# AI4Science-WestlakeU/cindm

Hardware: AMD Instinct MI355X
Metric: design samples/sec (1000-step DDPM, composed U-Nets); rel-err vs CPU ref (higher is better)
Workload: dtype f32; 1 GPU; nbody-2 TemporalUnet1D dim=64 horizon=24 attention, single model, batch 256/GPU, 1000 DDPM steps per design (BASELINE configs[1]); unet_evals_per_design=1000, reverse_steps_per_design=1000, parallelism=dp1 (design-sharded, one all-gather of final designs)

## Files before the change

### cindm_amd/csrc/cindm_hip.hip

```cpp
#include "kernels.h"
#include "kernels_dconv.h"
#include "kernels2d.h"
#include "kernels2d_v2.h"
#include "../../include/cindm_hip.h"

#include <hip/hip_ext.h>
#include <cmath>
#include <cstdio>
#include <cstdlib>
#include <cstring>
#include <map>
#include <mutex>
#include <string>
#include <unordered_map>
#include <vector>

using namespace cindm;

static thread_local std::string g_err;
static int fail(const std::string& m) { g_err = m; return -1; }
#define HIPCHK(x) do { hipError_t e_ = (x); if (e_ != hipSuccess) return fail(std::string(#x) + ": " + hipGetErrorString(e_)); } while (0)
#define REQUIRE(c, msg) do { if (!(c)) return fail(msg); } while (0)

extern "C" int cindm_abi_version(void) { return CINDM_ABI_VERSION; }
// ... 121 lines not shown
    const int mid = h->dims[nres];
    rtb("mid_block1", mid, mid);
    if (d.attention) attn("mid_attn", mid);
    rtb("mid_block2", mid, mid);
    cblock("final_conv.0", dim, dim);
    conv("final_conv.1", dim, d.transition_dim, 1);
    return 0;
}

static const OptDef kUnet1dOpts[] = {
    {"mfma_f32", 0, nullptr, OPT_PACK},
    {"local_gn", 1, "CINDM_LOCAL_GN", OPT_PACK},
    {"attn_site", 1, "CINDM_ATTN_SITE", OPT_PACK},
    {"level0", 1, "CINDM_LEVEL0", OPT_PACK},
    {"level1", 1, "CINDM_LEVEL1", OPT_PACK},
    {"ups_last", 1, "CINDM_UPS_LAST", OPT_PACK},
    {"ups_tail", 1, "CINDM_UPS_TAIL", OPT_PACK},
    {"level_pairs", 1, "CINDM_LEVEL_PAIRS", OPT_PACK},
    {"attn_head", 1, "CINDM_ATTN_HEAD", OPT_PACK},
    {"dconv", 1, "CINDM_DCONV", OPT_PACK},
    {"ws_alias", 1, "CINDM_WS_ALIAS", OPT_PACK},
    {"pingpong", 1, "CINDM_PINGPONG", OPT_PACK},
    {"dresample", 2, "CINDM_DRESAMPLE", OPT_PACK},
    {"dconv2", 1, "CINDM_DCONV2", OPT_PACK},
    {"l2_prefetch", 1, "CINDM_L2_PREFETCH", OPT_PACK},
    {"fuse_gather", 1, nullptr, OPT_PACK},
    {"fuse_update", 1, "CINDM_FUSE_UPDATE", OPT_PACK},
    {"taps", 0, "CINDM_TAPS", OPT_PACK},
    {"recover", 1, nullptr, OPT_RUNTIME},
    {"no_exchange", 0, "CINDM_NO_EXCHANGE", OPT_RUNTIME},
    {"tune", 0, "CINDM_TUNE", OPT_RUNTIME},
    {"stress", 0, "CINDM_STRESS", OPT_PACK},
    {"auto_range", 1, "CINDM_AUTO_RANGE", OPT_PACK},
    {"range_fallback", 0, nullptr, OPT_READONLY},
    {"dbg", 0, "CINDM_DBG", OPT_PACK},
};

static void unet1d_plan(cindm_unet1d* h);
extern "C" int cindm_unet1d_set_option(cindm_unet1d* h, const char* key, int32_t value) {
    const int rc = core_set_option(h, key, value);
    if (rc == 1) {
        h->generation = ++g_generation;
        if (std::string(key) == "tune" && h->finalized) unet1d_plan(h);
    }
    return rc < 0 ? -1 : 0;
}
// ... 597 lines not shown
    if (!identity && !h->packed.count(p + ".residual_conv#h3")) return false;
    const int k0 = x0.C / 128, k1 = x1 ? x1->C / 128 : 0;
    if (w0->second.CinP != (k0 + k1) * 128 || w1->second.CinP != cout || cout % 128) return false;
    return dconv_instantiated(L, k0, k1, !identity) && dconv_instantiated(L, cout / 128, 0, false);
}

static bool dconv2_instantiated(int L, int k0, int k1, bool res, int kb) {
    if (L == 6) return kb == 2 && ((k0 == 1 && k1 == 0 && res) || (k0 == 2 && k1 == 0 && !res) || (k0 == 2 && k1 == 2 && res));
    if (L == 3) return (kb == 4 && ((k0 == 2 && k1 == 0 && res) || (k0 == 4 && k1 == 0 && !res) || (k0 == 4 && k1 == 4 && res))) ||
                       (kb == 2 && k0 == 4 && k1 == 0 && res);
    return false;
}

static Ten emit_rtb_dconv2(Emitter& E, const std::string& p, const Ten& x0, const Ten* x1, int cout) {
    cindm_unet1d* h = E.h;
    const int Bp = (int)E.rows, L = x0.L, S = 48 / L, gw = cout / 8, NT = cout / 32;
    const int tiles = (Bp + S - 1) / S;
    const Packed& w0 = h->packed.at(p + ".blocks.0.block.0");
    const Packed& w1 = h->packed.at(p + ".blocks.1.block.0");
    const bool identity = !h->packed.count(p + ".residual_conv");
    const int k0 = x0.C / 128, k1 = x1 ? x1->C / 128 : 0, kb = cout / 128;
    Ten y0; y0.L = L; y0.C = cout; y0.ld = cout; E.planes(y0);
    Ten out = E.ten(L, cout); E.planes(out);
    unsigned long long* fl = E.xchg((size_t)tiles * NT);
    unsigned long long* xa = gw == 64 ? E.xchg((size_t)tiles * NT * 32) : nullptr;
    unsigned long long* xb = gw == 64 ? E.xchg((size_t)tiles * NT * 32) : nullptr;
    E.need_epoch();
    ++E.launches;
    {
        cindm_unet1d::WReg r{};
        const size_t t0 = w0.sz * 4 / (size_t)NT, t1 = w1.sz * 4 / (size_t)NT;
        int XS = NT / 4;
        while (XS >= 1 && XS < 8 && tiles % (8 / XS) != 0) XS *= 2;
        const bool remap = (XS == 2 || XS == 4) && NT % XS == 0 && tiles % (8 / XS) == 0;
        if (NT % 8 == 0 && !(h->O("tune") & 1)) {
            r.off[0] = w0.off * 4; r.bytes[0] = (unsigned)t0; r.stride[0] = (unsigned)t0;
            if (NT >= 16) { r.off[1] = w0.off * 4 + 8 * t0; r.bytes[1] = (unsigned)t0; r.stride[1] = (unsigned)t0; }
        }
        else if (NT % 8 == 0) { r.off[0] = w0.off * 4; r.bytes[0] = (unsigned)t0; r.stride[0] = (unsigned)t0;
                           r.off[1] = w1.off * 4; r.bytes[1] = (unsigned)t1; r.stride[1] = (unsigned)t1;
                         }
        else { r.off[0] = w0.off * 4; r.bytes[0] = (unsigned)std::min(w0.sz * 4, (size_t)2 << 20); }
        E.pf_issue = p != "downs.3.1";
        Pf pf; E.pf_step(pf, r);
        E.pf_issue = true;
        if (E.dry) { E.drop(y0); return out; }
        Dconv2Args d;
        std::memset(&d, 0, sizeof(d));
        d.pf = pf;
        auto src = [](DSrc& s, const Ten& t) { s.f32 = t.pl ? nullptr : t.p; s.planes = t.pl; s.pstride = t.pst; s.C = t.C; s.ld = t.ld; };
        src(d.src[0], x0); if (x1) src(d.src[1], *x1);
        d.Wa = reinterpret_cast<const uint4*>(E.W(w0)); d.bias_a = E.B(w0); d.ncha = w0.CinP / 128;
        d.Wb = reinterpret_cast<const uint4*>(E.W(w1)); d.bias_b = E.B(w1);
        if (!identity) {
            const Packed& rc = h->packed.at(p + ".residual_conv#h3");
            d.W2 = reinterpret_cast<const uint4*>(E.W(rc)); d.bias2 = E.B(rc);
        } else { d.res = x0.p; d.ldres = x0.ld; }
        d.Bp = Bp; d.N = cout; d.NT = NT; d.gw = gw;
        d.gamma_a = E.V(p + ".blocks.0.block.2.weight"); d.beta_a = E.V(p + ".blocks.0.block.2.bias");
        d.gamma_b = E.V(p + ".blocks.1.block.2.weight"); d.beta_b = E.V(p + ".blocks.1.block.2.bias");
        d.tb = h->ttable + h->tb_off.at(p); d.tb_ld = h->tb_ld; d.t_ptr = E.t_ptr; d.t_imm = E.t_imm;
        d.y0 = y0.pl; d.y0_pstride = y0.pst; d.flags = reinterpret_cast<unsigned*>(fl);
        d.out_f32 = out.p; d.ldo = out.ld; d.out_planes = out.pl; d.out_pstride = out.pst;
        d.xchg_a = xa; d.xchg_b = xb; d.epoch = h->ep(); d.err_flag = h->epoch_dev + 1;
        d.stress = h->O("stress"); d.dbg = h->O("dbg") >= 30 ? h->O("dbg") - 30 : 0;
        d.tune = h->O("tune");
        d.xs = remap ? XS : 0;
        d.ph = E.ph_next("dconv2<" + std::to_string(L) + "," + std::to_string(k0) + "," + std::to_string(k1) + "," + (identity ? "false" : "true") + "," +
                         std::to_string(kb) + "> " + p);
        const dim3 grid((unsigned)NT, (unsigned)tiles);
        const double cin = (double)x0.C + (x1 ? (double)x1->C : 0.0);
        E.prof_begin(4, 2.0 * Bp * L * cout * cin * (5.0 + (identity ? 0.0 : 1.0)) + 2.0 * Bp * L * cout * (double)cout * 5.0);
        if (E.prof) { E.prof->back().gx = grid.x; E.prof->back().gy = grid.y; E.prof->back().nstage = d.ncha + kb; }
#define DC2(L_, K0_, K1_, R_, KB_) KLAUNCH(E, (dconv2_kernel<L_, K0_, K1_, R_, KB_>), grid, dim3(256), 0, d)
        if (L == 6) {
            if (k0 == 1) DC2(6, 1, 0, true, 2);
            else if (k1 == 2) DC2(6, 2, 2, true, 2);
            else DC2(6, 2, 0, false, 2);
        } else {
            if (k0 == 2) DC2(3, 2, 0, true, 4);
            else if (k1 == 4) DC2(3, 4, 4, true, 4);
            else if (kb == 2) DC2(3, 4, 0, true, 2);
            else DC2(3, 4, 0, false, 4);
        }
#undef DC2
        E.prof_end();
        hipError_t e = hipGetLastError();
        if (e != hipSuccess && E.err == hipSuccess) E.err = e;
    }
    E.drop(y0);
    E.tap(p, out);
    return out;
}

static Ten emit_rtb_dconv(Emitter& E, const std::string& p, const Ten& x0, const Ten* x1, int cout) {
    cindm_unet1d* h = E.h;
    const int Bp = (int)E.rows, L = x0.L, S = 48 / L, gw = cout / 8, NT = cout / 32;
    const int tiles = (Bp + S - 1) / S;
    const Packed& w0 = h->packed.at(p + ".blocks.0.block.0");
    const Packed& w1 = h->packed.at(p + ".blocks.1.block.0");
    const bool identity = !h->packed.count(p + ".residual_conv");
    if (h->O("dconv2") && !h->NX() && dconv2_instantiated(L, x0.C / 128, x1 ? x1->C / 128 : 0, !identity, cout / 128) &&
        w0.CinP / 128 == x0.C / 128 + (x1 ? x1->C / 128 : 0))
        return emit_rtb_dconv2(E, p, x0, x1, cout);
// ... 1041 lines not shown
```

### cindm_amd/csrc/kernels_dconv.h

```cpp
#pragma once
#include "kernels.h"
#include <type_traits>

namespace cindm {

__device__ __forceinline__ int spin_bound(const int* err_flag, bool forced_short, int full_log2 = 20) {
    const int seen = err_flag ? uniform_word(err_flag) : 0;
    return (forced_short || seen) ? (1 << 8) : (1 << full_log2);
}

struct DSrc {
    const float* f32;
    const uint4* planes;
    size_t pstride;
    int C, ld;
};

struct DconvArgs {
    DSrc src[2];
    const uint4* W; const float* bias;
    int nch;
    int Bp, N, NT;
    int gw;
    const float* gamma; const float* beta;
// ... 360 lines not shown
            if (sok[q]) a.out2[(size_t)grow[q] * a.ldo2 + gn] = r2[q];
    }
    l2_prefetch_done(a.pf, pfr);
}


struct Dconv2Args {
    DSrc src[2];
    const uint4* Wa; const float* bias_a; int ncha;
    const uint4* Wb; const float* bias_b;
    const uint4* W2; const float* bias2;
    int Bp, N, NT, gw;
    const float* gamma_a; const float* beta_a; const float* gamma_b; const float* beta_b;
    const float* tb; int tb_ld; const int* t_ptr; int t_imm;
    const float* res; int ldres;
    uint4* y0; size_t y0_pstride;
    unsigned* flags;
    float* out_f32; int ldo; uint4* out_planes; size_t out_pstride;
    unsigned long long* xchg_a; unsigned long long* xchg_b; const int* epoch; int* err_flag;
    Pf pf; int stress; int dbg;
    PhaseBuf ph;
    int tune;
    int xs;
};

#ifdef CINDM_KPROF
#define PHK(i) PH(i)
#define PHX(i) do { } while (0)
#else
#define PHK(i) do { } while (0)
#define PHX(i) PH(i)
#endif
template <int L, int KPW0, int KPW1, bool RES, int KPWB>
__global__ __launch_bounds__(256) void dconv2_kernel(const Dconv2Args a) {
    constexpr int T = 5;
    constexpr int S = 48 / L, PB = 16 / S, H = PB - 1, RPAD = (L + 2 * H) * S, NWIN = L + H;
    constexpr int KPWA = KPW0 > KPW1 ? KPW0 : KPW1;
    constexpr int KPWM = KPWA > KPWB ? KPWA : KPWB;
    constexpr int KST = 4 * KPWM;
    constexpr int PLANE_U4 = KST * 4 * RPAD;
    static_assert(L == 3 || L == 6, "3 or 6 positions per sample");
    __shared__ uint4 Img[2][PLANE_U4];
    __shared__ float Red[4][TM * LDR];
    __shared__ uint4 Tile[2 * 48 * 5];

    PH_DECL;
    PH(0);
    const int t_now = step_scalar(a.t_ptr, a.t_imm);
    const unsigned tag = (unsigned)uniform_word(a.epoch);
    const int err_seen = uniform_word(a.err_flag);
    const int tid = threadIdx.x, lane = tid & 63, w = tid >> 6;
    int nt = blockIdx.x, mt = blockIdx.y;
#ifndef CINDM_NO_XCD_REMAP
    if (a.xs > 0) {
        const int XS = a.xs, bl = blockIdx.x + gridDim.x * blockIdx.y, xcd = bl & 7, sl = bl >> 3, q4 = gridDim.x / XS;
        nt = (sl % q4) * XS + (xcd & (XS - 1)); mt = (xcd / XS) + (8 / XS) * (sl / q4);
    }
#endif
    const int b0 = mt * S;
    const int ns = min(S, a.Bp - b0);
    const int n = tid & 31, rq = tid >> 5;
    const int gn = nt * TN + n;
    int grow[6];
    bool sok[6];
#pragma unroll
    for (int q = 0; q < 6; ++q) {
        const int pos = (S == 16) ? (q >> 1) : q;
        const int s = (S == 16) ? rq + 8 * (q & 1) : rq;
        sok[q] = s < ns;
        grow[q] = (b0 + min(s, ns - 1)) * L + pos;
    }

    struct Stg { const uint4* base[3]; size_t kstride, second; int slot[3]; bool f32; };
    auto stg_init = [&](const DSrc& s, Stg& g) {
        g.f32 = s.planes == nullptr;
#pragma unroll
        for (int i = 0; i < 3; ++i) {
            const int item = lane + 64 * i;
            if (!g.f32) {
                const int kq = item / 48, row = item - kq * 48;
                g.base[i] = s.planes + (size_t)mt * (s.C >> 5) * 192 + item;
                g.slot[i] = kq * RPAD + H * S + row;
            } else {
                const int row = item >> 2, kq = item & 3;
                const int sm = row % S, pos = row / S;
                g.base[i] = reinterpret_cast<const uint4*>(s.f32 + (size_t)((b0 + min(sm, ns - 1)) * L + pos) * s.ld + kq * 8);
                g.slot[i] = kq * RPAD + H * S + row;
            }
        }
        g.kstride = g.f32 ? 8 : 192;
        g.second = g.f32 ? 1 : s.pstride;
// ... 12 lines not shown
#pragma unroll
            for (int i = 0; i < 3; ++i) {
                const float4 v0 = __builtin_bit_cast(float4, raw[i][0]), v1 = __builtin_bit_cast(float4, raw[i][1]);
                const float v[8] = {v0.x, v0.y, v0.z, v0.w, v1.x, v1.y, v1.z, v1.w};
                half8 hi, lo;
#pragma unroll
                for (int e = 0; e < 8; ++e) {
                    hi[e] = (_Float16)v[e];
                    lo[e] = (_Float16)((v[e] - (float)hi[e]) * H3_SCALE);
                }
                Img[0][kb + slot[i]] = __builtin_bit_cast(uint4, hi);
                Img[1][kb + slot[i]] = __builtin_bit_cast(uint4, lo);
            }
        }
    };

    Stg g0, g1;
    stg_init(a.src[0], g0);
    uint4 raw0[KPW0][3][2];
#pragma unroll
    for (int j = 0; j < KPW0; ++j) load_raw(g0, j, raw0[j]);

    constexpr int BD = 1;
    half8 wr[BD][T][2][2];
    const uint4* wbase = a.Wa + (size_t)nt * a.ncha * (T * 4) * 256 + tid;
    const uint4* wbase_b = a.Wb + (size_t)nt * KPWB * (T * 4) * 256 + tid;
    auto load_b_tap = [&](const uint4* wb, int ch, int tap, auto slot_c) {
        constexpr int SL = decltype(slot_c)::value;
#if defined(CINDM_ABL) && (CINDM_ABL & 2)
        ch = 0;
#endif
        const uint4* wp = wb + ((size_t)ch * (T * 4) + tap * 4) * 256;
#pragma unroll
        for (int q = 0; q < 4; ++q) wr[SL][tap][q >> 1][q & 1] = __builtin_bit_cast(half8, wp[q * 256]);
    };
    constexpr std::integral_constant<int, 0> SLOT0{};
#pragma unroll
    for (int tap = 0; tap < T; ++tap) load_b_tap(wbase, 0, tap, SLOT0);
    half8 rreg[2][2];
    const uint4* rbase = a.W2 + (size_t)nt * a.ncha * 4 * 256 + tid;
    auto load_r = [&](int ch) {
        if constexpr (RES) {
            const uint4* wp = rbase + (size_t)ch * 4 * 256;
#pragma unroll
            for (int q = 0; q < 4; ++q) rreg[q >> 1][q & 1] = __builtin_bit_cast(half8, wp[q * 256]);
        }
    };
    load_r(0);
    uint4 raw1[KPW1 > 0 ? KPW1 : 1][3][2];
    if constexpr (KPW1 > 0) {
        stg_init(a.src[1], g1);
#pragma unroll
        for (int j = 0; j < KPW1; ++j) load_raw(g1, j, raw1[j]);
    }
    __builtin_amdgcn_sched_barrier(0);
    const int spin_cap = (a.dbg == 9 || err_seen) ? (1 << 8) : (1 << 20);
    const float gam_a = a.gamma_a[gn], bet_a = a.beta_a[gn], gam_b = a.gamma_b[gn], bet_b = a.beta_b[gn];
    const float bias_a_ld = (a.bias_a ? a.bias_a : a.gamma_a)[gn], bias_b_ld = (a.bias_b ? a.bias_b : a.gamma_a)[gn];
    const float tbv_ld = a.tb ? a.tb[(size_t)t_now * a.tb_ld + gn] : bias_a_ld;
    const float bias_a = a.bias_a ? bias_a_ld : 0.f, bias_b = a.bias_b ? bias_b_ld : 0.f, tbv = a.tb ? tbv_ld : 0.f;
    float bias2 = 0.f;
    if constexpr (RES) { const float b2 = (a.bias2 ? a.bias2 : a.gamma_a)[gn]; bias2 = a.bias2 ? b2 : 0.f; }
    float rs[6] = {0.f, 0.f, 0.f, 0.f, 0.f, 0.f};
    if constexpr (!RES) {
#pragma unroll
        for (int q = 0; q < 6; ++q) rs[q] = a.res[(size_t)grow[q] * a.ldres + gn];
    }
    __builtin_amdgcn_sched_barrier(0);
    PH(1);

    if constexpr (H > 0) {
        const uint4 z = {0u, 0u, 0u, 0u};
        for (int i = lane; i < KPWM * 4 * 2 * H * S; i += 64) {
            const int blk = i / (2 * H * S), r = i - blk * (2 * H * S);
            const int ks = 4 * (blk >> 2) + w, kq = blk & 3;
            const int row = r < H * S ? r : (L + H) * S + (r - H * S);
            Img[0][(ks * 4 + kq) * RPAD + row] = z;
            Img[1][(ks * 4 + kq) * RPAD + row] = z;
        }
    }

    f32x4 accM[3][2], accL[3][2], accRM[3][2], accRL[3][2];
    auto zero_acc = [&]() {
#pragma unroll
        for (int i = 0; i < 3; ++i)
#pragma unroll
            for (int j = 0; j < 2; ++j) { accM[i][j] = (f32x4){0.f, 0.f, 0.f, 0.f}; accL[i][j] = (f32x4){0.f, 0.f, 0.f, 0.f}; }
    };
    zero_acc();
#pragma unroll
    for (int i = 0; i < 3; ++i)
#pragma unroll
        for (int j = 0; j < 2; ++j) { accRM[i][j] = (f32x4){0.f, 0.f, 0.f, 0.f}; accRL[i][j] = (f32x4){0.f, 0.f, 0.f, 0.f}; }

    auto kstep = [&](const uint4* wb, int j, int chn, auto pf, auto ride, auto slot_c) {
        constexpr bool PF = decltype(pf)::value;
        constexpr bool RIDE = decltype(ride)::value;
        constexpr int SL = decltype(slot_c)::value;
        const int base = ((4 * j + w) * 4 + (lane >> 4)) * RPAD + (lane & 15);
        half8 fh[NWIN], fl[NWIN];
#pragma unroll
        for (int p = 0; p < NWIN; ++p) {
            fh[p] = __builtin_bit_cast(half8, Img[0][base + p * S]);
            fl[p] = __builtin_bit_cast(half8, Img[1][base + p * S]);
        }
#pragma unroll
        for (int tap = 0; tap < T; ++tap) {
#pragma unroll
            for (int mb = 0; mb < 3; ++mb) {
                const int p = mb * PB + tap - 2 + H;
                if (p < 0 || p >= NWIN) continue;
#if defined(CINDM_ABL) && (CINDM_ABL & 1)
#pragma unroll
                for (int nb = 0; nb < 2; ++nb)
#pragma unroll
                    for (int pl = 0; pl < 2; ++pl) {
                        const uint4 u = __builtin_bit_cast(uint4, wr[SL][tap][nb][pl]);
                        asm volatile("" :: "v"(u.x), "v"(u.y), "v"(u.z), "v"(u.w));
                    }
                {
                    const uint4 u = __builtin_bit_cast(uint4, fh[p]), u2 = __builtin_bit_cast(uint4, fl[p]);
                    asm volatile("" :: "v"(u.x), "v"(u.y), "v"(u.z), "v"(u.w), "v"(u2.x), "v"(u2.y), "v"(u2.z), "v"(u2.w));
                }
#else
#pragma unroll
                for (int nb = 0; nb < 2; ++nb) {
                    accM[mb][nb] = __builtin_amdgcn_mfma_f32_16x16x32_f16(fh[p], wr[SL][tap][nb][0], accM[mb][nb], 0, 0, 0);
                    accL[mb][nb] = __builtin_amdgcn_mfma_f32_16x16x32_f16(fh[p], wr[SL][tap][nb][1], accL[mb][nb], 0, 0, 0);
                }
#pragma unroll
                for (int nb = 0; nb < 2; ++nb)
                    accL[mb][nb] = __builtin_amdgcn_mfma_f32_16x16x32_f16(fl[p], wr[SL][tap][nb][0], accL[mb][nb], 0, 0, 0);
#endif
            }
            if constexpr (RIDE) if (tap == 2) {
#pragma unroll
                for (int mb = 0; mb < 3; ++mb) {
                    const int p = mb * PB + H;
#pragma unroll
                    for (int nb = 0; nb < 2; ++nb) {
                        accRM[mb][nb] = __builtin_amdgcn_mfma_f32_16x16x32_f16(fh[p], rreg[nb][0], accRM[mb][nb], 0, 0, 0);
                        accRL[mb][nb] = __builtin_amdgcn_mfma_f32_16x16x32_f16(fh[p], rreg[nb][1], accRL[mb][nb], 0, 0, 0);
                    }
#pragma unroll
                    for (int nb = 0; nb < 2; ++nb)
                        accRL[mb][nb] = __builtin_amdgcn_mfma_f32_16x16x32_f16(fl[p], rreg[nb][0], accRL[mb][nb], 0, 0, 0);
                }
                if constexpr (PF) load_r(chn);
            }
            if constexpr (PF) {
                load_b_tap(wb, chn, tap, slot_c);
                __builtin_amdgcn_sched_barrier(0);
            }
        }
    };
    constexpr std::true_type YES{};
    constexpr std::false_type NO{};
    constexpr std::integral_constant<bool, RES> RIDE_A{};
    if constexpr (KPW1 == 0) {
#pragma unroll
        for (int j = 0; j < KPW0 - 1; ++j) { store_raw(g0.f32, g0.slot, j, raw0[j]); PHK(2 + 2 * j); kstep(wbase, j, j + 1, YES, RIDE_A, SLOT0); PHK(3 + 2 * j); }
        store_raw(g0.f32, g0.slot, KPW0 - 1, raw0[KPW0 - 1]);
        PHK(2 + 2 * (KPW0 - 1));
        kstep(wbase, KPW0 - 1, 0, NO, RIDE_A, SLOT0);
        PHK(3 + 2 * (KPW0 - 1));
    } else {
#pragma unroll
        for (int j = 0; j < KPW0; ++j) { store_raw(g0.f32, g0.slot, j, raw0[j]); kstep(wbase, j, j + 1, YES, RIDE_A, SLOT0); }
#pragma unroll
        for (int j = 0; j < KPW1 - 1; ++j) { store_raw(g1.f32, g1.slot, j, raw1[j]); kstep(wbase, j, KPW0 + j + 1, YES, RIDE_A, SLOT0); }
        store_raw(g1.f32, g1.slot, KPW1 - 1, raw1[KPW1 - 1]);
        kstep(wbase, KPW1 - 1, 0, NO, RIDE_A, SLOT0);
    }
    PHX(2);
    PfRegs pfr;
#pragma unroll
    for (int k = 0; k < PF_REGIONS; ++k) pfr.v[k][0] = pfr.v[k][1] = 0u;
    auto issue_b = [&]() {
#pragma unroll
        for (int tap = 0; tap < T; ++tap) load_b_tap(wbase_b, 0, tap, SLOT0);
        __builtin_amdgcn_sched_barrier(0);
    };

    auto reduce_to = [&](const f32x4 (&m)[3][2], const f32x4 (&l)[3][2], float bs, float (&v)[6]) {
#pragma unroll
        for (int mb = 0; mb < 3; ++mb)
#pragma unroll
            for (int nb = 0; nb < 2; ++nb)
#pragma unroll
                for (int rg = 0; rg < 4; ++rg)
                    Red[w][(mb * 16 + (lane >> 4) * 4 + rg) * LDR + nb * 16 + (lane & 15)] = m[mb][nb][rg] + l[mb][nb][rg] * H3_INV;
        __syncthreads();
#pragma unroll
        for (int q = 0; q < 6; ++q) {
            const int r = rq + 8 * q;
            v[q] = ((Red[0][r * LDR + n] + Red[1][r * LDR + n]) + (Red[2][r * LDR + n] + Red[3][r * LDR + n])) + bs;
        }
    };
    constexpr int NSAMP = (S == 16) ? 2 : 1;
    const int gwt = a.gw < TN ? a.gw : TN;
    const float cnt = (float)(L * gwt);
    auto gn_mish = [&](const float (&v)[6], unsigned long long* xchg, float gam, float bet, float (&y)[6], auto phb, auto after_xchg) {
        constexpr int PHB = decltype(phb)::value;
        (void)PHB;
        float mean[NSAMP], rstd[NSAMP];
#pragma unroll
        for (int js = 0; js < NSAMP; ++js) {
            float s1 = 0.f;
#pragma unroll
            for (int pos = 0; pos < L; ++pos) s1 += v[(S == 16) ? 2 * pos + js : pos];
            s1 = row16_sum(s1);
            if (gwt == 32) s1 = xsum16(s1);
            const float m = s1 / cnt;
            float s2 = 0.f;
#pragma unroll
            for (int pos = 0; pos < L; ++pos) { const float d = v[(S == 16) ? 2 * pos + js : pos] - m; s2 += d * d; }
            s2 = row16_sum(s2);
            if (gwt == 32) s2 = xsum16(s2);
            mean[js] = m; rstd[js] = s2;
        }
        if (a.gw == 64) {
            stress_delay(a.stress, 1u);
            const int sbase = ((mt * a.NT + nt) * 16) * 2, pbase = ((mt * a.NT + (nt ^ 1)) * 16) * 2;
#pragma unroll
            for (int js = 0; js < NSAMP; ++js) {
                const int s = (S == 16) ? rq + 8 * js : rq;
                if (n == 0) {
                    const unsigned long long q0 = ((unsigned long long)tag << 32) | __builtin_bit_cast(unsigned, mean[js]);
                    const unsigned long long q1 = ((unsigned long long)tag << 32) | __builtin_bit_cast(unsigned, rstd[js]);
                    __hip_atomic_store(xchg + sbase + s * 2, q0, __ATOMIC_RELAXED, __HIP_MEMORY_SCOPE_AGENT);
                    __hip_atomic_store(xchg + sbase + s * 2 + 1, q1, __ATOMIC_RELAXED, __HIP_MEMORY_SCOPE_AGENT);
                }
            }
            stress_delay(a.stress, 2u);
            PHX(PHB);
            unsigned long long gq[NSAMP][2];
            {
                int spins = 0;
                while (true) {
                    bool ok = true;
#pragma unroll
                    for (int js = 0; js < NSAMP; ++js) {
                        const int s = (S == 16) ? rq + 8 * js : rq;
                        gq[js][0] = __hip_atomic_load(xchg + pbase + s * 2, __ATOMIC_RELAXED, __HIP_MEMORY_SCOPE_AGENT);
// ... 2 lines not shown
#pragma unroll
                    for (int js = 0; js < NSAMP; ++js) ok = ok & ((unsigned)(gq[js][0] >> 32) == tag) & ((unsigned)(gq[js][1] >> 32) == tag);
                    if (__all(ok)) break;
                    if (++spins > spin_cap) { if (lane == 0) atomicExch(a.err_flag, 1); break; }
                    __builtin_amdgcn_s_sleep(2);
                }
            }
#pragma unroll
            for (int js = 0; js < NSAMP; ++js) {
                const unsigned long long q0 = gq[js][0], q1 = gq[js][1];
                const float mp = __builtin_bit_cast(float, (unsigned)q0), M2p = __builtin_bit_cast(float, (unsigned)q1);
                const float m = 0.5f * (mean[js] + mp);
                const float d0 = mean[js] - m, d1 = mp - m;
                mean[js] = m;
                rstd[js] = (rstd[js] + M2p) + cnt * (d0 * d0 + d1 * d1);
            }
            PHX(PHB + 1);
        }
        after_xchg();
        const float cnt_all = a.gw == 64 ? 2.f * cnt : cnt;
#pragma unroll
        for (int js = 0; js < NSAMP; ++js) rstd[js] = 1.0f / sqrtf(rstd[js] / cnt_all + 1e-5f);
#pragma unroll
        for (int q = 0; q < 6; ++q) {
            const int js = (S == 16) ? (q & 1) : 0;
            y[q] = mish_f((v[q] - mean[js]) * rstd[js] * gam + bet);
        }
    };
    constexpr int TP = 20;
    auto planes_to_tile = [&](const float (&y)[6]) {
        uint32_t* tw = reinterpret_cast<uint32_t*>(Tile);
#pragma unroll
        for (int q = 0; q < 6; ++q) {
            const int r = rq + 8 * q;
            const _Float16 hi = (_Float16)y[q];
            const _Float16 lo = (_Float16)((y[q] - (float)hi) * H3_SCALE);
            const uint32_t own = (uint32_t)__builtin_bit_cast(uint16_t, hi) | ((uint32_t)__builtin_bit_cast(uint16_t, lo) << 16);
            const uint32_t nbr = (uint32_t)__builtin_amdgcn_update_dpp(0, (int)own, 0xB1, 0xf, 0xf, false);
            const bool odd = n & 1;
            const uint32_t word = odd ? ((nbr >> 16) | (own & 0xffff0000u)) : ((own & 0xffffu) | (nbr << 16));
            tw[(odd ? 48 * TP : 0) + r * TP + (n >> 1)] = word;
        }
    };

    float v[6], y[6];
    stress_delay(a.stress, 3u);
    reduce_to(accM, accL, bias_a, v);
    PHX(3);
    gn_mish(v, a.xchg_a, gam_a, bet_a, y, std::integral_constant<int, 4>{}, [&]() {});
#pragma unroll
    for (int q = 0; q < 6; ++q) y[q] += tbv;
    planes_to_tile(y);
    stress_delay(a.stress, 4u);
    __syncthreads();
    {
        const uint32_t* tw = reinterpret_cast<const uint32_t*>(Tile);
        const size_t plane_bytes = a.y0_pstride * 16;
        const auto rsrc = __builtin_amdgcn_make_buffer_rsrc(reinterpret_cast<void*>(a.y0), 0, (unsigned)(2 * plane_bytes), 0x00020000);
        auto store_item = [&](int i) {
            const int pl = i >= 192 ? 1 : 0, within = i - pl * 192;
            const int kq = within / 48, row = within - kq * 48;
            const uint4 t4 = *reinterpret_cast<const uint4*>(tw + pl * 48 * TP + row * TP + kq * 4);
            const unsigned off = (unsigned)(pl * plane_bytes + (((size_t)mt * a.NT + nt) * 192 + within) * 16);
            typedef unsigned int u32x4 __attribute__((ext_vector_type(4)));
            __builtin_amdgcn_raw_buffer_store_b128(__builtin_bit_cast(u32x4, t4), rsrc, off, 0, 16);
        };
        for (int i = tid; i < 384; i += 256) store_item(i);
        PHX(6);
        asm volatile("s_waitcnt vmcnt(0)" ::: "memory");
        stress_delay(a.stress, 6u);
        __syncthreads();
        if (tid == 0 && !(a.dbg == 9 && (nt & 1)))
            __hip_atomic_store(a.flags + 2 * ((size_t)mt * a.NT + nt), tag, __ATOMIC_RELAXED, __HIP_MEMORY_SCOPE_AGENT);
        PHX(7);
        issue_b();
        if (a.tune & 1) l2_prefetch(a.pf, pfr);
    }
    float r2[6] = {0.f, 0.f, 0.f, 0.f, 0.f, 0.f};
    if constexpr (RES) { reduce_to(accRM, accRL, bias2, r2); __syncthreads(); }
    PHX(8);

    constexpr int YB = KPWB < 2 ? KPWB : 2;
    uint4 rawb[YB][3][2];
    int slotb[3];
#pragma unroll
    for (int i = 0; i < 3; ++i) { const int item = lane + 64 * i, kq = item / 48, row = item - kq * 48; slotb[i] = kq * RPAD + H * S + row; }
    const size_t y0_plane_bytes = a.y0_pstride * 16;
    const auto y0_rsrc = __builtin_amdgcn_make_buffer_rsrc(reinterpret_cast<void*>(a.y0), 0, (unsigned)(2 * y0_plane_bytes), 0x00020000);
    auto fetch_y0 = [&](int j, uint4 (&dst)[3][2]) {
#pragma unroll
        for (int i = 0; i < 3; ++i) {
            const unsigned off = (unsigned)((((size_t)mt * a.NT + 4 * j + w) * 192 + lane + 64 * i) * 16);
            dst[i][0] = __builtin_bit_cast(uint4, __builtin_amdgcn_raw_buffer_load_b128(y0_rsrc, off, 0, 16));
            dst[i][1] = __builtin_bit_cast(uint4, __builtin_amdgcn_raw_buffer_load_b128(y0_rsrc, off + (unsigned)y0_plane_bytes, 0, 16));
        }
    };
    {
        stress_delay(a.stress, 7u);
        int spins = 0;
        const int spin_max = spin_cap;
        while (true) {
            unsigned fw[KPWB];
#pragma unroll
            for (int j = 0; j < KPWB; ++j)
                fw[j] = __hip_atomic_load(a.flags + 2 * ((size_t)mt * a.NT + 4 * j + w), __ATOMIC_RELAXED, __HIP_MEMORY_SCOPE_AGENT);
            bool ok = true;
#pragma unroll
            for (int j = 0; j < KPWB; ++j) ok = ok & (fw[j] == tag);
            if (ok) break;
            if (++spins > spin_max) { if (lane == 0) atomicExch(a.err_flag, 1); break; }
            __builtin_amdgcn_s_sleep(1);
        }
        asm volatile("" ::: "memory");
        PHX(9);
#pragma unroll
        for (int j = 0; j < YB; ++j) fetch_y0(j, rawb[j]);
        __builtin_amdgcn_sched_barrier(0);
    }
    zero_acc();
    auto kb_step = [&](auto jc) {
        constexpr int j = decltype(jc)::value;
        constexpr std::integral_constant<int, j % BD> slot{};
        store_raw(false, slotb, j, rawb[j % YB]);
        if (j + YB < KPWB) fetch_y0(j + YB, rawb[j % YB]);
        __builtin_amdgcn_sched_barrier(0);
        if constexpr (j + BD < KPWB) kstep(wbase_b, j, j + BD, YES, NO, slot);
        else kstep(wbase_b, j, 0, NO, NO, slot);
        __builtin_amdgcn_sched_barrier(0);
    };
    kb_step(std::integral_constant<int, 0>{});
    if constexpr (KPWB > 1) kb_step(std::integral_constant<int, 1>{});
    if constexpr (KPWB > 2) kb_step(std::integral_constant<int, 2>{});
    if constexpr (KPWB > 3) kb_step(std::integral_constant<int, 3>{});
    static_assert(KPWB <= 4, "phase B: at most four k-steps per wave");
    PHX(10);
    if (!(a.tune & 1)) l2_prefetch(a.pf, pfr);

    stress_delay(a.stress, 8u);
    reduce_to(accM, accL, bias_b, v);
    PHX(11);
    gn_mish(v, a.xchg_b, gam_b, bet_b, y, std::integral_constant<int, 12>{}, [&]() {});
#pragma unroll
    for (int q = 0; q < 6; ++q) y[q] += RES ? r2[q] : rs[q];
    if (a.out_f32 && a.pf.wt) {
        float ta[4] = {y[0], y[1], y[2], y[3]}, tb[4] = {y[4], y[5], 0.f, 0.f};
        quad_transpose4(ta, lane);
        quad_transpose4(tb, lane);
        const int j = lane & 3;
        const size_t c4 = (size_t)(gn & ~3);
        auto row_ok = [&](int q, int& g) { const int pos = (S == 16) ? (q >> 1) : q; const int sm = (S == 16) ? rq + 8 * (q & 1) : rq; g = (b0 + min(sm, ns - 1)) * L + pos; return sm < ns; };
        int g0; const bool ok0 = row_ok(j, g0);
        if (ok0) st_out4(a.out_f32, (size_t)g0 * a.ldo + c4, make_float4(ta[0], ta[1], ta[2], ta[3]), 1);
        if (j < 2) { int g1; if (row_ok(4 + j, g1)) st_out4(a.out_f32, (size_t)g1 * a.ldo + c4, make_float4(tb[0], tb[1], tb[2], tb[3]), 1); }
    } else {
#pragma unroll
        for (int q = 0; q < 6; ++q)
            if (a.out_f32 && sok[q]) st_out(a.out_f32, (size_t)grow[q] * a.ldo + gn, y[q], 0);
    }
    if (a.out_planes) {
        __syncthreads();
        planes_to_tile(y);
        __syncthreads();
        const uint32_t* tw = reinterpret_cast<const uint32_t*>(Tile);
        for (int i = tid; i < 384; i += 256) {
            const int pl = i >= 192 ? 1 : 0, within = i - pl * 192;
            const int kq = within / 48, row = within - kq * 48;
            const uint4 t4 = *reinterpret_cast<const uint4*>(tw + pl * 48 * TP + row * TP + kq * 4);
            st_out4(a.out_planes, pl * a.out_pstride + ((size_t)mt * a.NT + nt) * 192 + within, t4, a.pf.wt);
        }
    }
    PHX(14);
    l2_prefetch_done(a.pf, pfr);
    PH_FLUSH(a.ph);
}


struct DresArgs {
    const float* x; int ld;
    const uint4* W; const float* bias; int nch;
    int Bp, N, NT;
    float* out_f32; int ldo;
    uint4* out_planes; size_t out_pstride;
    Pf pf;
    PhaseBuf ph;
    int xs;
};

template <bool UP, int KPW, int NH>
__global__ __launch_bounds__(256) void dresample_kernel(const DresArgs a) {
// ... 455 lines not shown
```

Before: 845.0 samples/s.

## Split L=3 dconv2 blocks into 16-column halves with cross-block GroupNorm exchange

Adds an NH=2 form of the fused double-conv kernel for the L=3, single-source, 1x1-residual case. Each 32-column tile is split across two workgroups, doubling the grid when it stays within 256 blocks. The halves combine GroupNorm statistics through a tagged atomic exchange in global memory, and the final output is written by a keeper half using partner values sent via new exchange buffers. The aim is more parallelism for an under-filled layer, at the cost of extra global-memory spin-waits and exchange traffic.

```diff
diff --git a/cindm_amd/csrc/cindm_hip.hip b/cindm_amd/csrc/cindm_hip.hip
--- a/cindm_amd/csrc/cindm_hip.hip
+++ b/cindm_amd/csrc/cindm_hip.hip
@@ -167,6 +167,7 @@
     {"ws_alias", 1, "CINDM_WS_ALIAS", OPT_PACK},
     {"pingpong", 1, "CINDM_PINGPONG", OPT_PACK},
     {"dresample", 2, "CINDM_DRESAMPLE", OPT_PACK},
+    {"dconv2_split", 1, "CINDM_DCONV2_SPLIT", OPT_PACK},
     {"dconv2", 1, "CINDM_DCONV2", OPT_PACK},
     {"l2_prefetch", 1, "CINDM_L2_PREFETCH", OPT_PACK},
     {"fuse_gather", 1, nullptr, OPT_PACK},
@@ -810,17 +811,21 @@
     const int k0 = x0.C / 128, k1 = x1 ? x1->C / 128 : 0, kb = cout / 128;
     Ten y0; y0.L = L; y0.C = cout; y0.ld = cout; E.planes(y0);
     Ten out = E.ten(L, cout); E.planes(out);
-    unsigned long long* fl = E.xchg((size_t)tiles * NT);
-    unsigned long long* xa = gw == 64 ? E.xchg((size_t)tiles * NT * 32) : nullptr;
-    unsigned long long* xb = gw == 64 ? E.xchg((size_t)tiles * NT * 32) : nullptr;
+    const bool split = h->O("dconv2_split") && L == 3 && k0 == 4 && k1 == 0 && kb == 2 && !identity && gw == 32 && 2 * NT * tiles <= 256;
+    const int NH = split ? 2 : 1;
+    unsigned long long* fl = E.xchg((size_t)tiles * NT * NH);
+    unsigned long long* xa = gw == 64 || split ? E.xchg((size_t)tiles * NT * NH * 32) : nullptr;
+    unsigned long long* xb = gw == 64 || split ? E.xchg((size_t)tiles * NT * NH * 32) : nullptr;
+    unsigned long long* xv = split ? E.xchg((size_t)tiles * NT * NH * 3 * 128) : nullptr;
+    unsigned long long* xr = split ? E.xchg((size_t)tiles * NT * NH * 3 * 128) : nullptr;
     E.need_epoch();
     ++E.launches;
     {
         cindm_unet1d::WReg r{};
         const size_t t0 = w0.sz * 4 / (size_t)NT, t1 = w1.sz * 4 / (size_t)NT;
-        int XS = NT / 4;
+        int XS = NH * NT / 4;
         while (XS >= 1 && XS < 8 && tiles % (8 / XS) != 0) XS *= 2;
-        const bool remap = (XS == 2 || XS == 4) && NT % XS == 0 && tiles % (8 / XS) == 0;
+        const bool remap = (XS == 2 || XS == 4) && (NH * NT) % XS == 0 && tiles % (8 / XS) == 0 && (!split || XS == 4);
         if (NT % 8 == 0 && !(h->O("tune") & 1)) {
             r.off[0] = w0.off * 4; r.bytes[0] = (unsigned)t0; r.stride[0] = (unsigned)t0;
             if (NT >= 16) { r.off[1] = w0.off * 4 + 8 * t0; r.bytes[1] = (unsigned)t0; r.stride[1] = (unsigned)t0; }
@@ -854,9 +859,10 @@
         d.stress = h->O("stress"); d.dbg = h->O("dbg") >= 30 ? h->O("dbg") - 30 : 0;
         d.tune = h->O("tune");
         d.xs = remap ? XS : 0;
+        d.xchg_v = xv; d.xchg_r = xr;
         d.ph = E.ph_next("dconv2<" + std::to_string(L) + "," + std::to_string(k0) + "," + std::to_string(k1) + "," + (identity ? "false" : "true") + "," +
                          std::to_string(kb) + "> " + p);
-        const dim3 grid((unsigned)NT, (unsigned)tiles);
+        const dim3 grid((unsigned)(NH * NT), (unsigned)tiles);
         const double cin = (double)x0.C + (x1 ? (double)x1->C : 0.0);
         E.prof_begin(4, 2.0 * Bp * L * cout * cin * (5.0 + (identity ? 0.0 : 1.0)) + 2.0 * Bp * L * cout * (double)cout * 5.0);
         if (E.prof) { E.prof->back().gx = grid.x; E.prof->back().gy = grid.y; E.prof->back().nstage = d.ncha + kb; }
@@ -868,6 +874,7 @@
         } else {
             if (k0 == 2) DC2(3, 2, 0, true, 4);
             else if (k1 == 4) DC2(3, 4, 4, true, 4);
+            else if (kb == 2 && split) KLAUNCH(E, (dconv2_kernel<3, 4, 0, true, 2, 2>), grid, dim3(256), 0, d);
             else if (kb == 2) DC2(3, 4, 0, true, 2);
             else DC2(3, 4, 0, false, 4);
         }
diff --git a/cindm_amd/csrc/kernels_dconv.h b/cindm_amd/csrc/kernels_dconv.h
--- a/cindm_amd/csrc/kernels_dconv.h
+++ b/cindm_amd/csrc/kernels_dconv.h
@@ -406,7 +406,21 @@
     PhaseBuf ph;
     int tune;
     int xs;
+    unsigned long long* xchg_v; unsigned long long* xchg_r;
 };
+
+__device__ __forceinline__ void merge_halves(float m0, float M0, float m1, float M1, float cnt, float& mean, float& M2) {
+    const float m = 0.5f * (m0 + m1);
+    const float d0 = m0 - m, d1 = m1 - m;
+    mean = m;
+    M2 = (M0 + M1) + cnt * (d0 * d0 + d1 * d1);
+}
+__device__ __forceinline__ void row_pair(float own, bool odd_row, float& v0, float& v1) {
+    float p, q;
+    permlane16_pair(own, p, q);
+    const float other = __builtin_bit_cast(unsigned, p) == __builtin_bit_cast(unsigned, own) ? q : p;
+    v0 = odd_row ? other : own; v1 = odd_row ? own : other;
+}
 
 #ifdef CINDM_KPROF
 #define PHK(i) PH(i)
@@ -415,7 +429,7 @@
 #define PHK(i) do { } while (0)
 #define PHX(i) PH(i)
 #endif
-template <int L, int KPW0, int KPW1, bool RES, int KPWB>
+template <int L, int KPW0, int KPW1, bool RES, int KPWB, int NH = 1>
 __global__ __launch_bounds__(256) void dconv2_kernel(const Dconv2Args a) {
     constexpr int T = 5;
     constexpr int S = 48 / L, PB = 16 / S, H = PB - 1, RPAD = (L + 2 * H) * S, NWIN = L + H;
@@ -424,6 +438,8 @@
     constexpr int KST = 4 * KPWM;
     constexpr int PLANE_U4 = KST * 4 * RPAD;
     static_assert(L == 3 || L == 6, "3 or 6 positions per sample");
+    constexpr int NBW = 2 / NH, TNW = TN / NH, RQN = 256 / TNW, NQ = TM / RQN;
+    static_assert(NH == 1 || (NH == 2 && L == 3 && RES && KPW1 == 0), "16-column form: L = 3 blocks with a riding 1x1, one source");
     __shared__ uint4 Img[2][PLANE_U4];
     __shared__ float Red[4][TM * LDR];
     __shared__ uint4 Tile[2 * 48 * 5];
@@ -441,16 +457,22 @@
         nt = (sl % q4) * XS + (xcd & (XS - 1)); mt = (xcd / XS) + (8 / XS) * (sl / q4);
     }
 #endif
+    int hb = 0;
+    if constexpr (NH == 2) {
+        const int hx = nt;
+        hb = hx & 1;
+        nt = a.xs == 4 ? ((hx >> 1) & 1) * 2 + ((hx >> 2) & 1) + 4 * (hx >> 3) : hx >> 1;
+    }
     const int b0 = mt * S;
     const int ns = min(S, a.Bp - b0);
-    const int n = tid & 31, rq = tid >> 5;
-    const int gn = nt * TN + n;
-    int grow[6];
-    bool sok[6];
-#pragma unroll
-    for (int q = 0; q < 6; ++q) {
-        const int pos = (S == 16) ? (q >> 1) : q;
-        const int s = (S == 16) ? rq + 8 * (q & 1) : rq;
+    const int n = tid & (TNW - 1), rq = tid / TNW;
+    const int gn = nt * TN + hb * TNW + n;
+    int grow[NQ];
+    bool sok[NQ];
+#pragma unroll
+    for (int q = 0; q < NQ; ++q) {
+        const int pos = (S == 16 && NH == 1) ? (q >> 1) : q;
+        const int s = (S == 16 && NH == 1) ? rq + 8 * (q & 1) : rq;
         sok[q] = s < ns;
         grow[q] = (b0 + min(s, ns - 1)) * L + pos;
     }
@@ -509,7 +531,7 @@
     for (int j = 0; j < KPW0; ++j) load_raw(g0, j, raw0[j]);
 
     constexpr int BD = 1;
-    half8 wr[BD][T][2][2];
+    half8 wr[BD][T][NBW][2];
     const uint4* wbase = a.Wa + (size_t)nt * a.ncha * (T * 4) * 256 + tid;
     const uint4* wbase_b = a.Wb + (size_t)nt * KPWB * (T * 4) * 256 + tid;
     auto load_b_tap = [&](const uint4* wb, int ch, int tap, auto slot_c) {
@@ -519,18 +541,18 @@
 #endif
         const uint4* wp = wb + ((size_t)ch * (T * 4) + tap * 4) * 256;
 #pragma unroll
-        for (int q = 0; q < 4; ++q) wr[SL][tap][q >> 1][q & 1] = __builtin_bit_cast(half8, wp[q * 256]);
+        for (int q = 0; q < 2 * NBW; ++q) wr[SL][tap][q >> 1][q & 1] = __builtin_bit_cast(half8, wp[(NH == 2 ? hb * 2 + q : q) * 256]);
     };
     constexpr std::integral_constant<int, 0> SLOT0{};
 #pragma unroll
     for (int tap = 0; tap < T; ++tap) load_b_tap(wbase, 0, tap, SLOT0);
-    half8 rreg[2][2];
+    half8 rreg[NBW][2];
     const uint4* rbase = a.W2 + (size_t)nt * a.ncha * 4 * 256 + tid;
     auto load_r = [&](int ch) {
         if constexpr (RES) {
             const uint4* wp = rbase + (size_t)ch * 4 * 256;
 #pragma unroll
-            for (int q = 0; q < 4; ++q) rreg[q >> 1][q & 1] = __builtin_bit_cast(half8, wp[q * 256]);
+            for (int q = 0; q < 2 * NBW; ++q) rreg[q >> 1][q & 1] = __builtin_bit_cast(half8, wp[(NH == 2 ? hb * 2 + q : q) * 256]);
         }
     };
     load_r(0);
@@ -548,10 +570,14 @@
     const float bias_a = a.bias_a ? bias_a_ld : 0.f, bias_b = a.bias_b ? bias_b_ld : 0.f, tbv = a.tb ? tbv_ld : 0.f;
     float bias2 = 0.f;
     if constexpr (RES) { const float b2 = (a.bias2 ? a.bias2 : a.gamma_a)[gn]; bias2 = a.bias2 ? b2 : 0.f; }
-    float rs[6] = {0.f, 0.f, 0.f, 0.f, 0.f, 0.f};
+    float rs[NQ];
+#pragma unroll
+    for (int q = 0; q < NQ; ++q) rs[q] = 0.f;
+    float gam_bp = 0.f, bet_bp = 0.f;
+    if constexpr (NH == 2) { const int gnp = nt * TN + (hb ^ 1) * TNW + n; gam_bp = a.gamma_b[gnp]; bet_bp = a.beta_b[gnp]; }
     if constexpr (!RES) {
 #pragma unroll
-        for (int q = 0; q < 6; ++q) rs[q] = a.res[(size_t)grow[q] * a.ldres + gn];
+        for (int q = 0; q < NQ; ++q) rs[q] = a.res[(size_t)grow[q] * a.ldres + gn];
     }
     __builtin_amdgcn_sched_barrier(0);
     PH(1);
@@ -567,18 +593,18 @@
         }
     }
 
-    f32x4 accM[3][2], accL[3][2], accRM[3][2], accRL[3][2];
+    f32x4 accM[3][NBW], accL[3][NBW], accRM[3][NBW], accRL[3][NBW];
     auto zero_acc = [&]() {
 #pragma unroll
         for (int i = 0; i < 3; ++i)
 #pragma unroll
-            for (int j = 0; j < 2; ++j) { accM[i][j] = (f32x4){0.f, 0.f, 0.f, 0.f}; accL[i][j] = (f32x4){0.f, 0.f, 0.f, 0.f}; }
+            for (int j = 0; j < NBW; ++j) { accM[i][j] = (f32x4){0.f, 0.f, 0.f, 0.f}; accL[i][j] = (f32x4){0.f, 0.f, 0.f, 0.f}; }
     };
     zero_acc();
 #pragma unroll
     for (int i = 0; i < 3; ++i)
 #pragma unroll
-        for (int j = 0; j < 2; ++j) { accRM[i][j] = (f32x4){0.f, 0.f, 0.f, 0.f}; accRL[i][j] = (f32x4){0.f, 0.f, 0.f, 0.f}; }
+        for (int j = 0; j < NBW; ++j) { accRM[i][j] = (f32x4){0.f, 0.f, 0.f, 0.f}; accRL[i][j] = (f32x4){0.f, 0.f, 0.f, 0.f}; }
 
     auto kstep = [&](const uint4* wb, int j, int chn, auto pf, auto ride, auto slot_c) {
         constexpr bool PF = decltype(pf)::value;
@@ -599,7 +625,7 @@
                 if (p < 0 || p >= NWIN) continue;
 #if defined(CINDM_ABL) && (CINDM_ABL & 1)
 #pragma unroll
-                for (int nb = 0; nb < 2; ++nb)
+                for (int nb = 0; nb < NBW; ++nb)
 #pragma unroll
                     for (int pl = 0; pl < 2; ++pl) {
                         const uint4 u = __builtin_bit_cast(uint4, wr[SL][tap][nb][pl]);
@@ -611,12 +637,12 @@
                 }
 #else
 #pragma unroll
-                for (int nb = 0; nb < 2; ++nb) {
+                for (int nb = 0; nb < NBW; ++nb) {
                     accM[mb][nb] = __builtin_amdgcn_mfma_f32_16x16x32_f16(fh[p], wr[SL][tap][nb][0], accM[mb][nb], 0, 0, 0);
                     accL[mb][nb] = __builtin_amdgcn_mfma_f32_16x16x32_f16(fh[p], wr[SL][tap][nb][1], accL[mb][nb], 0, 0, 0);
                 }
 #pragma unroll
-                for (int nb = 0; nb < 2; ++nb)
+                for (int nb = 0; nb < NBW; ++nb)
                     accL[mb][nb] = __builtin_amdgcn_mfma_f32_16x16x32_f16(fl[p], wr[SL][tap][nb][0], accL[mb][nb], 0, 0, 0);
 #endif
             }
@@ -625,12 +651,12 @@
                 for (int mb = 0; mb < 3; ++mb) {
                     const int p = mb * PB + H;
 #pragma unroll
-                    for (int nb = 0; nb < 2; ++nb) {
+                    for (int nb = 0; nb < NBW; ++nb) {
                         accRM[mb][nb] = __builtin_amdgcn_mfma_f32_16x16x32_f16(fh[p], rreg[nb][0], accRM[mb][nb], 0, 0, 0);
                         accRL[mb][nb] = __builtin_amdgcn_mfma_f32_16x16x32_f16(fh[p], rreg[nb][1], accRL[mb][nb], 0, 0, 0);
                     }
 #pragma unroll
-                    for (int nb = 0; nb < 2; ++nb)
+                    for (int nb = 0; nb < NBW; ++nb)
                         accRL[mb][nb] = __builtin_amdgcn_mfma_f32_16x16x32_f16(fl[p], rreg[nb][0], accRL[mb][nb], 0, 0, 0);
                 }
                 if constexpr (PF) load_r(chn);
@@ -669,44 +695,115 @@
         __builtin_amdgcn_sched_barrier(0);
     };
 
-    auto reduce_to = [&](const f32x4 (&m)[3][2], const f32x4 (&l)[3][2], float bs, float (&v)[6]) {
+    auto reduce_to = [&](const f32x4 (&m)[3][NBW], const f32x4 (&l)[3][NBW], float bs, float (&v)[NQ]) {
 #pragma unroll
         for (int mb = 0; mb < 3; ++mb)
 #pragma unroll
-            for (int nb = 0; nb < 2; ++nb)
+            for (int nb = 0; nb < NBW; ++nb)
 #pragma unroll
                 for (int rg = 0; rg < 4; ++rg)
                     Red[w][(mb * 16 + (lane >> 4) * 4 + rg) * LDR + nb * 16 + (lane & 15)] = m[mb][nb][rg] + l[mb][nb][rg] * H3_INV;
         __syncthreads();
 #pragma unroll
-        for (int q = 0; q < 6; ++q) {
-            const int r = rq + 8 * q;
+        for (int q = 0; q < NQ; ++q) {
+            const int r = rq + RQN * q;
             v[q] = ((Red[0][r * LDR + n] + Red[1][r * LDR + n]) + (Red[2][r * LDR + n] + Red[3][r * LDR + n])) + bs;
         }
     };
-    constexpr int NSAMP = (S == 16) ? 2 : 1;
+    constexpr int NSAMP = (S == 16 && NH == 1) ? 2 : 1;
     const int gwt = a.gw < TN ? a.gw : TN;
     const float cnt = (float)(L * gwt);
-    auto gn_mish = [&](const float (&v)[6], unsigned long long* xchg, float gam, float bet, float (&y)[6], auto phb, auto after_xchg) {
+    const bool halfwise = NH == 2 || a.gw == 32;
+    const float cnt_h = (float)(L * 16);
+    const bool keeper = NH == 2 && (rq >> 3) == hb;
+    const int xslot = (mt * a.NT + nt) * 2;
+    const int lidx = (rq & 7) * 16 + n;
+    float ypart[NQ];
+    float r2[NQ];
+#pragma unroll
+    for (int q = 0; q < NQ; ++q) { ypart[q] = 0.f; r2[q] = 0.f; }
+    auto gn_mish = [&](const float (&v)[NQ], unsigned long long* xchg, float gam, float bet, float (&y)[NQ], auto phb, auto after_xchg, auto lines) {
         constexpr int PHB = decltype(phb)::value;
+        constexpr bool LINES = decltype(lines)::value;
         (void)PHB;
         float mean[NSAMP], rstd[NSAMP];
 #pragma unroll
         for (int js = 0; js < NSAMP; ++js) {
             float s1 = 0.f;
 #pragma unroll
-            for (int pos = 0; pos < L; ++pos) s1 += v[(S == 16) ? 2 * pos + js : pos];
+            for (int pos = 0; pos < L; ++pos) s1 += v[(S == 16 && NH == 1) ? 2 * pos + js : pos];
             s1 = row16_sum(s1);
-            if (gwt == 32) s1 = xsum16(s1);
-            const float m = s1 / cnt;
+            if (!halfwise && gwt == 32) s1 = xsum16(s1);
+            const float m = s1 / (halfwise ? cnt_h : cnt);
             float s2 = 0.f;
 #pragma unroll
-            for (int pos = 0; pos < L; ++pos) { const float d = v[(S == 16) ? 2 * pos + js : pos] - m; s2 += d * d; }
+            for (int pos = 0; pos < L; ++pos) { const float d = v[(S == 16 && NH == 1) ? 2 * pos + js : pos] - m; s2 += d * d; }
             s2 = row16_sum(s2);
-            if (gwt == 32) s2 = xsum16(s2);
+            if (!halfwise && gwt == 32) s2 = xsum16(s2);
             mean[js] = m; rstd[js] = s2;
-        }
-        if (a.gw == 64) {
+            if (NH == 1 && halfwise) {
+                const bool odd_row = (n >> 4) & 1;
+                float m0, m1, M0, M1;
+                row_pair(m, odd_row, m0, m1);
+                row_pair(s2, odd_row, M0, M1);
+                merge_halves(m0, M0, m1, M1, cnt_h, mean[js], rstd[js]);
+            }
+        }
+        if constexpr (NH == 2) {
+            stress_delay(a.stress, 1u);
+            const int sbase = (xslot + hb) * 32, pbase = (xslot + (hb ^ 1)) * 32;
+            if (n == 0) {
+                const unsigned long long q0 = ((unsigned long long)tag << 32) | __builtin_bit_cast(unsigned, mean[0]);
+                const unsigned long long q1 = ((unsigned long long)tag << 32) | __builtin_bit_cast(unsigned, rstd[0]);
+                __hip_atomic_store(xchg + sbase + rq * 2, q0, __ATOMIC_RELAXED, __HIP_MEMORY_SCOPE_AGENT);
+                __hip_atomic_store(xchg + sbase + rq * 2 + 1, q1, __ATOMIC_RELAXED, __HIP_MEMORY_SCOPE_AGENT);
+            }
+            if constexpr (LINES) if (!keeper) {
+#pragma unroll
+                for (int q = 0; q < NQ; ++q)
+                    __hip_atomic_store(a.xchg_v + ((size_t)(xslot + hb) * NQ + q) * 128 + lidx, ((unsigned long long)tag << 32) | __builtin_bit_cast(unsigned, v[q]),
+                                       __ATOMIC_RELAXED, __HIP_MEMORY_SCOPE_AGENT);
+            }
+            stress_delay(a.stress, 2u);
+            PHX(PHB);
+            const bool wantl = LINES && keeper;
+            unsigned long long gq[2], gv[NQ], gr[NQ];
+#pragma unroll
+            for (int q = 0; q < NQ; ++q) gv[q] = gr[q] = 0ull;
+            {
+                int spins = 0;
+                while (true) {
+                    gq[0] = __hip_atomic_load(xchg + pbase + rq * 2, __ATOMIC_RELAXED, __HIP_MEMORY_SCOPE_AGENT);
+                    gq[1] = __hip_atomic_load(xchg + pbase + rq * 2 + 1, __ATOMIC_RELAXED, __HIP_MEMORY_SCOPE_AGENT);
+                    bool ok = ((unsigned)(gq[0] >> 32) == tag) & ((unsigned)(gq[1] >> 32) == tag);
+                    if (wantl) {
+#pragma unroll
+                        for (int q = 0; q < NQ; ++q) {
+                            const size_t o = ((size_t)(xslot + (hb ^ 1)) * NQ + q) * 128 + lidx;
+                            gv[q] = __hip_atomic_load(a.xchg_v + o, __ATOMIC_RELAXED, __HIP_MEMORY_SCOPE_AGENT);
+                            gr[q] = __hip_atomic_load(a.xchg_r + o, __ATOMIC_RELAXED, __HIP_MEMORY_SCOPE_AGENT);
+                        }
+#pragma unroll
+                        for (int q = 0; q < NQ; ++q) ok = ok & ((unsigned)(gv[q] >> 32) == tag) & ((unsigned)(gr[q] >> 32) == tag);
+                    }
+                    if (__all(ok)) break;
+                    if (++spins > spin_cap) { if (lane == 0) atomicExch(a.err_flag, 1); break; }
+                    __builtin_amdgcn_s_sleep(2);
+                }
+            }
+            const float mp = __builtin_bit_cast(float, (unsigned)gq[0]), M2p = __builtin_bit_cast(float, (unsigned)gq[1]);
+            const float mo = mean[0], M2o = rstd[0];
+            if (hb == 0) merge_halves(mo, M2o, mp, M2p, cnt_h, mean[0], rstd[0]);
+            else merge_halves(mp, M2p, mo, M2o, cnt_h, mean[0], rstd[0]);
+            if (wantl) {
+                const float rs_ = 1.0f / sqrtf(rstd[0] / cnt + 1e-5f);
+#pragma unroll
+                for (int q = 0; q < NQ; ++q)
+                    ypart[q] = mish_f((__builtin_bit_cast(float, (unsigned)gv[q]) - mean[0]) * rs_ * gam_bp + bet_bp) + __builtin_bit_cast(float, (unsigned)gr[q]);
+            }
+            PHX(PHB + 1);
+        }
+        if (NH == 1 && a.gw == 64) {
             stress_delay(a.stress, 1u);
             const int sbase = ((mt * a.NT + nt) * 16) * 2, pbase = ((mt * a.NT + (nt ^ 1)) * 16) * 2;
 #pragma unroll
@@ -755,17 +852,17 @@
 #pragma unroll
         for (int js = 0; js < NSAMP; ++js) rstd[js] = 1.0f / sqrtf(rstd[js] / cnt_all + 1e-5f);
 #pragma unroll
-        for (int q = 0; q < 6; ++q) {
-            const int js = (S == 16) ? (q & 1) : 0;
+        for (int q = 0; q < NQ; ++q) {
+            const int js = (S == 16 && NH == 1) ? (q & 1) : 0;
             y[q] = mish_f((v[q] - mean[js]) * rstd[js] * gam + bet);
         }
     };
     constexpr int TP = 20;
-    auto planes_to_tile = [&](const float (&y)[6]) {
+    auto planes_to_tile = [&](const float (&y)[NQ]) {
         uint32_t* tw = reinterpret_cast<uint32_t*>(Tile);
 #pragma unroll
-        for (int q = 0; q < 6; ++q) {
-            const int r = rq + 8 * q;
+        for (int q = 0; q < NQ; ++q) {
+            const int r = rq + RQN * q;
             const _Float16 hi = (_Float16)y[q];
             const _Float16 lo = (_Float16)((y[q] - (float)hi) * H3_SCALE);
             const uint32_t own = (uint32_t)__builtin_bit_cast(uint16_t, hi) | ((uint32_t)__builtin_bit_cast(uint16_t, lo) << 16);
@@ -776,13 +873,21 @@
         }
     };
 
-    float v[6], y[6];
+    auto tile_item = [&](int i, int& pl, int& within, int& kq, int& row) {
+        constexpr int PER = 192 / NH;
+        pl = i >= PER ? 1 : 0;
+        const int wl = i - pl * PER;
+        kq = wl / 48; row = wl - kq * 48;
+        within = (NH == 2 ? 2 * hb * 48 : 0) + wl;
+    };
+
+    float v[NQ], y[NQ];
     stress_delay(a.stress, 3u);
     reduce_to(accM, accL, bias_a, v);
     PHX(3);
-    gn_mish(v, a.xchg_a, gam_a, bet_a, y, std::integral_constant<int, 4>{}, [&]() {});
-#pragma unroll
-    for (int q = 0; q < 6; ++q) y[q] += tbv;
+    gn_mish(v, a.xchg_a, gam_a, bet_a, y, std::integral_constant<int, 4>{}, [&]() {}, NO);
+#pragma unroll
+    for (int q = 0; q < NQ; ++q) y[q] += tbv;
     planes_to_tile(y);
     stress_delay(a.stress, 4u);
     __syncthreads();
@@ -791,26 +896,31 @@
         const size_t plane_bytes = a.y0_pstride * 16;
         const auto rsrc = __builtin_amdgcn_make_buffer_rsrc(reinterpret_cast<void*>(a.y0), 0, (unsigned)(2 * plane_bytes), 0x00020000);
         auto store_item = [&](int i) {
-            const int pl = i >= 192 ? 1 : 0, within = i - pl * 192;
-            const int kq = within / 48, row = within - kq * 48;
+            int pl, within, kq, row;
+            tile_item(i, pl, within, kq, row);
             const uint4 t4 = *reinterpret_cast<const uint4*>(tw + pl * 48 * TP + row * TP + kq * 4);
             const unsigned off = (unsigned)(pl * plane_bytes + (((size_t)mt * a.NT + nt) * 192 + within) * 16);
             typedef unsigned int u32x4 __attribute__((ext_vector_type(4)));
             __builtin_amdgcn_raw_buffer_store_b128(__builtin_bit_cast(u32x4, t4), rsrc, off, 0, 16);
         };
-        for (int i = tid; i < 384; i += 256) store_item(i);
+        for (int i = tid; i < 384 / NH; i += 256) store_item(i);
         PHX(6);
         asm volatile("s_waitcnt vmcnt(0)" ::: "memory");
         stress_delay(a.stress, 6u);
         __syncthreads();
         if (tid == 0 && !(a.dbg == 9 && (nt & 1)))
-            __hip_atomic_store(a.flags + 2 * ((size_t)mt * a.NT + nt), tag, __ATOMIC_RELAXED, __HIP_MEMORY_SCOPE_AGENT);
+            __hip_atomic_store(a.flags + 2 * (((size_t)mt * a.NT + nt) * NH + hb), tag, __ATOMIC_RELAXED, __HIP_MEMORY_SCOPE_AGENT);
         PHX(7);
         issue_b();
         if (a.tune & 1) l2_prefetch(a.pf, pfr);
     }
-    float r2[6] = {0.f, 0.f, 0.f, 0.f, 0.f, 0.f};
     if constexpr (RES) { reduce_to(accRM, accRL, bias2, r2); __syncthreads(); }
+    if constexpr (NH == 2) if (!keeper) {
+#pragma unroll
+        for (int q = 0; q < NQ; ++q)
+            __hip_atomic_store(a.xchg_r + ((size_t)(xslot + hb) * NQ + q) * 128 + lidx, ((unsigned long long)tag << 32) | __builtin_bit_cast(unsigned, r2[q]),
+                               __ATOMIC_RELAXED, __HIP_MEMORY_SCOPE_AGENT);
+    }
     PHX(8);
 
     constexpr int YB = KPWB < 2 ? KPWB : 2;
@@ -833,13 +943,13 @@
         int spins = 0;
         const int spin_max = spin_cap;
         while (true) {
-            unsigned fw[KPWB];
-#pragma unroll
-            for (int j = 0; j < KPWB; ++j)
-                fw[j] = __hip_atomic_load(a.flags + 2 * ((size_t)mt * a.NT + 4 * j + w), __ATOMIC_RELAXED, __HIP_MEMORY_SCOPE_AGENT);
+            unsigned fw[KPWB * NH];
+#pragma unroll
+            for (int j = 0; j < KPWB * NH; ++j)
+                fw[j] = __hip_atomic_load(a.flags + 2 * (((size_t)mt * a.NT + 4 * (j / NH) + w) * NH + j % NH), __ATOMIC_RELAXED, __HIP_MEMORY_SCOPE_AGENT);
             bool ok = true;
 #pragma unroll
-            for (int j = 0; j < KPWB; ++j) ok = ok & (fw[j] == tag);
+            for (int j = 0; j < KPWB * NH; ++j) ok = ok & (fw[j] == tag);
             if (ok) break;
             if (++spins > spin_max) { if (lane == 0) atomicExch(a.err_flag, 1); break; }
             __builtin_amdgcn_s_sleep(1);
@@ -872,10 +982,23 @@
     stress_delay(a.stress, 8u);
     reduce_to(accM, accL, bias_b, v);
     PHX(11);
-    gn_mish(v, a.xchg_b, gam_b, bet_b, y, std::integral_constant<int, 12>{}, [&]() {});
-#pragma unroll
-    for (int q = 0; q < 6; ++q) y[q] += RES ? r2[q] : rs[q];
-    if (a.out_f32 && a.pf.wt) {
+    gn_mish(v, a.xchg_b, gam_b, bet_b, y, std::integral_constant<int, 12>{}, [&]() {}, std::integral_constant<bool, NH == 2>{});
+#pragma unroll
+    for (int q = 0; q < NQ; ++q) y[q] += RES ? r2[q] : rs[q];
+    if constexpr (NH == 2) {
+        if (a.out_f32 && keeper) {
+            float ta[4] = {y[0], y[1], y[2], ypart[0]}, tb[4] = {ypart[1], ypart[2], 0.f, 0.f};
+            quad_transpose4(ta, lane);
+            quad_transpose4(tb, lane);
+            const int j = lane & 3;
+            const size_t c_own = (size_t)(gn & ~3), c_par = (size_t)((nt * TN + (hb ^ 1) * TNW + n) & ~3);
+            const size_t srow = (size_t)(b0 + min(rq, ns - 1)) * L;
+            if (rq < ns) {
+                st_out4(a.out_f32, (srow + (j < 3 ? j : 0)) * a.ldo + (j < 3 ? c_own : c_par), make_float4(ta[0], ta[1], ta[2], ta[3]), a.pf.wt);
+                if (j < 2) st_out4(a.out_f32, (srow + 1 + j) * a.ldo + c_par, make_float4(tb[0], tb[1], tb[2], tb[3]), a.pf.wt);
+            }
+        }
+    } else if (a.out_f32 && a.pf.wt) {
         float ta[4] = {y[0], y[1], y[2], y[3]}, tb[4] = {y[4], y[5], 0.f, 0.f};
         quad_transpose4(ta, lane);
         quad_transpose4(tb, lane);
@@ -887,7 +1010,7 @@
         if (j < 2) { int g1; if (row_ok(4 + j, g1)) st_out4(a.out_f32, (size_t)g1 * a.ldo + c4, make_float4(tb[0], tb[1], tb[2], tb[3]), 1); }
     } else {
 #pragma unroll
-        for (int q = 0; q < 6; ++q)
+        for (int q = 0; q < NQ; ++q)
             if (a.out_f32 && sok[q]) st_out(a.out_f32, (size_t)grow[q] * a.ldo + gn, y[q], 0);
     }
     if (a.out_planes) {
@@ -895,9 +1018,9 @@
         planes_to_tile(y);
         __syncthreads();
         const uint32_t* tw = reinterpret_cast<const uint32_t*>(Tile);
-        for (int i = tid; i < 384; i += 256) {
-            const int pl = i >= 192 ? 1 : 0, within = i - pl * 192;
-            const int kq = within / 48, row = within - kq * 48;
+        for (int i = tid; i < 384 / NH; i += 256) {
+            int pl, within, kq, row;
+            tile_item(i, pl, within, kq, row);
             const uint4 t4 = *reinterpret_cast<const uint4*>(tw + pl * 48 * TP + row * TP + kq * 4);
             st_out4(a.out_planes, pl * a.out_pstride + ((size_t)mt * a.NT + nt) * 192 + within, t4, a.pf.wt);
         }
```

Result: no change. 848.1 samples/s (median of 6 runs) (+0.4%).
